# nju-websoft/OpenEA

Hardware: AMD Instinct MI355X
Metric: training triples/sec (k=10 truncated negatives + limited loss + Adagrad) (higher is better)
Workload: dtype f32; 1 GPU; BootEA/AlignE translational step, EN-FR-100K-V1 shape (synthetic), dim=100, GLOBAL batch=20000 positives (weak scaling: 20000 per GPU x 1 GPU), k=10, truncated eps=0.98; the same workload at every N (; global_batch=20000, entities=200000, parallelism=single

## Files before the change

include/openea_hip.h:

```cpp
#ifndef OPENEA_HIP_H
#define OPENEA_HIP_H

#include <stddef.h>
#include <stdint.h>

#ifdef __cplusplus
extern "C" {
#endif

#define OEA_OK 0
#define OEA_EINVAL (-1)
#define OEA_EHIP (-2)
#define OEA_ENOMEM (-3)
#define OEA_EUNSUPPORTED (-4)

int oea_version(void);
const char *oea_last_error(void);
int oea_device_count(void);

int oea_profile_begin(int32_t stride);
int oea_profile_end(int32_t group, double *out_ms_host, int32_t *n_calls_host);

typedef struct oea_store *oea_store_t;
int oea_store_create(int64_t rows, int32_t dim, oea_store_t *out);
// ... 298 lines not shown
    double *loss_accum;
} oea_epoch;
int oea_triple_epoch_range(const oea_epoch *e, int32_t step_begin, int32_t step_end, int32_t rank, int32_t world, void *plan,
                           size_t plan_bytes, int32_t plan_built, void *stream);

size_t oea_epoch_layout_bytes(int64_t n);
int oea_epoch_layout(const int32_t *triples, int64_t n1, int64_t n2, const int64_t *slot, int64_t n_slots, uint64_t seed, uint32_t epoch,
                     int32_t *dall, void *workspace, size_t ws_bytes, void *stream);

int32_t oea_step_plan_supported(const oea_step_cfg *cfg, int64_t n_ent, int64_t n_rel, int32_t ld, int32_t k);
size_t oea_step_plan_bytes(int64_t n_total, int32_t steps, int64_t max_batch, int64_t n_ent, int32_t ld);
int oea_step_plan_build(const int32_t *pos_all, const int32_t *neg_all, int32_t k, const int64_t *offsets_dev, int64_t n_total,
                        int32_t steps, int64_t max_batch, int64_t n_ent, int32_t ld, void *plan, size_t plan_bytes, void *stream);
int oea_step_plan_offsets(int64_t n_total, int32_t steps, int64_t max_batch, int64_t n_ent, int32_t ld, int64_t *out);
int oea_step_plan_rel_order_offset(int64_t n_total, int32_t steps, int64_t max_batch, int64_t n_ent, int32_t ld, int64_t *out);

struct oea_comm;
int oea_triple_epoch_range_comm(struct oea_comm *comm, const oea_epoch *e, int32_t step_begin, int32_t step_end, void *send, void *own,
                                void *rel_x, float *upd, float *all, void *stream);


uint32_t oea_perm_index(uint32_t i, uint32_t n, uint32_t key);
int oea_sample_link_negatives(const int32_t *pos_links, int64_t n_pos, int32_t k, const int32_t *ents1, int32_t n1,
                              const int32_t *ents2, int32_t n2, const int32_t *nbr1, const int32_t *row1,
                              const int32_t *nbr2, const int32_t *row2, int32_t nbr_k, const uint64_t *exclude,
                              uint64_t exclude_cap, uint64_t seed, uint32_t step, int32_t *out_pairs, float *out_valid,
                              uint64_t *scratch_keys, int32_t *scratch_vals, uint64_t scratch_cap, void *stream);

int oea_greedy_matching(const int32_t *left, const int32_t *right, const float *weight, int64_t n_edges,
                        uint8_t *selected);
// ... 243 lines not shown
```

openea_amd/_lib.py:

```python
import ctypes as C
import os

_HERE = os.path.dirname(os.path.abspath(__file__))
DETERMINISTIC = os.environ.get("OEA_STEP_DETERMINISTIC", "0")[:1] == "1"
LIB_PATH = os.environ.get("OPENEA_HIP_LIB") or os.path.join(_HERE, "csrc",
                                                            "libopenea_hip_det.so" if DETERMINISTIC else "libopenea_hip.so")


class OpenEAHipError(RuntimeError):
    pass


class StepCfg(C.Structure):
    _fields_ = [("loss_kind", C.c_int32), ("l1", C.c_int32), ("margin", C.c_float),
                ("pos_margin", C.c_float), ("neg_margin", C.c_float), ("balance", C.c_float),
                ("ent_l2_norm", C.c_int32), ("rel_l2_norm", C.c_int32), ("opt_kind", C.c_int32),
                ("lr", C.c_float), ("neg_group_k", C.c_int32), ("score_kind", C.c_int32),
                ("normal", C.c_void_p), ("normal_acc", C.c_void_p),
                ("ent_transfer_base", C.c_int32), ("rel_transfer_base", C.c_int32),
                ("beta1", C.c_float), ("beta2", C.c_float), ("eps", C.c_float), ("opt_t", C.c_int32)]


class SamplerSide(C.Structure):
    _fields_ = [("table", C.c_void_p), ("capacity", C.c_uint64), ("entity_list", C.c_void_p),
# ... 117 lines not shown
                                       _u32, _u32, _i32, _vp, _vp, _vp]),
    "oea_sample_negatives_replay": (C.c_int, [_vp, _i64, _i32, _vp, _u64, _vp, _i32, _vp, _vp, _i32, _i32, _vp, _vp, _vp, _vp]),
    "oea_tripleset_filter_bits": (C.c_uint64, [_u64]),
    "oea_tripleset_filter_build": (C.c_int, [_vp, _i64, _vp, _u64, _vp]),
    "oea_sample_negatives_pair": (C.c_int, [_vp, _i64, _i64, _i32, C.POINTER(SamplerSide), C.POINTER(SamplerSide),
                                            _u64, _u32, _u32, _i32, _vp, _vp, _vp]),
    "oea_sample_negatives_epoch": (C.c_int, [_vp, _i64, _vp, _vp, _i32, _i32, C.POINTER(SamplerSide),
                                             C.POINTER(SamplerSide), _u64, _u32, _i32, _vp, _vp, _vp]),
    "oea_triple_epoch_range": (C.c_int, [C.POINTER(Epoch), _i32, _i32, _i32, _i32, _vp, _sz, _i32, _vp]),
    "oea_epoch_layout_bytes": (_sz, [_i64]),
    "oea_epoch_layout": (C.c_int, [_vp, _i64, _i64, _vp, _i64, _u64, _u32, _vp, _vp, _sz, _vp]),
    "oea_step_plan_supported": (_i32, [C.POINTER(StepCfg), _i64, _i64, _i32, _i32]),
    "oea_step_plan_bytes": (_sz, [_i64, _i32, _i64, _i64, _i32]),
    "oea_step_plan_offsets": (C.c_int, [_i64, _i32, _i64, _i64, _i32, _vp]),
    "oea_step_plan_rel_order_offset": (C.c_int, [_i64, _i32, _i64, _i64, _i32, _vp]),
    "oea_step_plan_build": (C.c_int, [_vp, _vp, _i32, _vp, _i64, _i32, _i64, _i64, _i32, _vp, _sz, _vp]),
    "oea_triple_epoch_range_comm": (C.c_int, [_vp, C.POINTER(Epoch), _i32, _i32, _vp, _vp, _vp, _vp, _vp, _vp]),
    "oea_rotate_workspace_bytes": (_sz, [_i64, _i64, _i32]),
    "oea_rotate_exchange_doubles": (_sz, [_i64, _i64, _i32]),
    "oea_rotate_step": (C.c_int, [_vp, _vp, _i64, _vp, _vp, _i64, _i32, _i32, _vp, _i64, _vp, _i64, _i32,
                                  C.POINTER(RotateCfg), _vp, _vp, _i32, _vp]),
    "oea_rotate_lookup": (C.c_int, [_vp, _i64, _i32, _i32, _vp, _i64, _i32, _i32, _vp, _i32, _vp]),
    "oea_mapping_workspace_floats": (_sz, [_i64, _i32, _i32]),
    "oea_mapping_step": (C.c_int, [_vp, _i32, _i32, _i32, _vp, _vp, _i64, _vp, _vp, C.c_float, C.c_float, _i32, _vp, _vp,
                                   _vp, _vp, _vp]),
    "oea_mapping_epoch": (C.c_int, [_vp, _vp, _i64, _vp, _vp, _i64, _i32, _i32, _i32, _vp, _i32, _i64, _vp, _vp, _f32, _f32, _i32,
                                    C.POINTER(StepCfg), _vp, _vp, _vp, _vp, _vp]),
    "oea_sea_mapping_workspace_floats": (_sz, [_i64, _i64, _i32, _i32]),
    "oea_sea_mapping_step": (C.c_int, [_vp, _i32, _i32, _vp, _vp, _i64, _vp, _vp, _i64, _vp, _vp, _vp, _f32, _f32, C.POINTER(StepCfg),
                                       _vp, _vp, _vp, _vp, _vp]),
# ... 187 lines not shown
```

openea_amd/csrc/step_plan.h:

```cpp
#pragma once
#include <hip/hip_runtime.h>
#include <stddef.h>
#include <stdint.h>

namespace oea {

struct StepPlanView {
    uint64_t *keys_a, *keys_b;
    uint32_t *vals_a, *vals_b;
    uint64_t *ukeys;
    uint32_t *ucount;
    uint32_t *uoff;
    int32_t *n_unique;
    int32_t *step_first;
    uint32_t *pflags;
    uint4 *recs;
    uint8_t *inplan;
    float *contrib;
    void *temp;
    size_t temp_bytes;
    uint32_t *rel_order;
    int row_bits;
};

constexpr uint32_t kPlanHubEntries = 8;

size_t step_plan_layout(int64_t n_total, int32_t steps, int64_t max_batch, int64_t n_ent, int32_t ld, void *base, StepPlanView *v);

}
```

openea_amd/csrc/step_plan.hip:

```cpp
#include <string.h>

#include <rocprim/rocprim.hpp>

#include <algorithm>

#include "common.h"
#include "step_plan.h"

namespace oea {

static size_t al256(size_t x) { return (x + 255) / 256 * 256; }
static int bits_for(uint64_t max_value) { int b = 1; while (b < 64 && (max_value >> b) != 0) ++b; return b; }

size_t step_plan_layout(int64_t n_total, int32_t steps, int64_t max_batch, int64_t n_ent, int32_t ld, void *base, StepPlanView *v) {
    const size_t m = (size_t)std::max<int64_t>(2 * n_total, 1);
    size_t off = 0;
    char *b = static_cast<char *>(base);
    auto take = [&](size_t bytes) { size_t o = off; off += al256(bytes); return b ? b + o : nullptr; };
    StepPlanView w{};
    w.keys_a = (uint64_t *)take(8 * m);
    w.keys_b = (uint64_t *)take(8 * m);
    w.vals_a = (uint32_t *)take(4 * m);
    w.vals_b = (uint32_t *)take(4 * m);
    w.ukeys = (uint64_t *)take(8 * m);
// ... 4 lines not shown
    w.pflags = (uint32_t *)take(4 * (size_t)std::max<int64_t>(n_total, 1));
    w.recs = (uint4 *)take(16 * m);
    w.inplan = (uint8_t *)take((size_t)std::max<int32_t>(steps, 1) * (size_t)n_ent);
    w.contrib = (float *)take(sizeof(float) * 2 * (size_t)std::max<int64_t>(max_batch, 1) * (size_t)ld);
    size_t t1 = 0, t2 = 0, t3 = 0;
    (void)rocprim::radix_sort_pairs(nullptr, t1, (const uint64_t *)nullptr, (uint64_t *)nullptr, (const uint32_t *)nullptr,
                                    (uint32_t *)nullptr, m, 0, 64, (hipStream_t)0);
    (void)rocprim::run_length_encode(nullptr, t2, (const uint64_t *)nullptr, m, (uint64_t *)nullptr, (uint32_t *)nullptr,
                                     (int32_t *)nullptr, (hipStream_t)0);
    (void)rocprim::exclusive_scan(nullptr, t3, (const uint32_t *)nullptr, (uint32_t *)nullptr, 0u, m + 1, rocprim::plus<uint32_t>(),
                                  (hipStream_t)0);
    const size_t n1 = (size_t)std::max<int64_t>(n_total, 1);
    w.temp_bytes = std::max(std::max(t1, std::max(t2, t3)), al256(4 * n1)) + 256;
    w.temp = take(w.temp_bytes);
    w.rel_order = (uint32_t *)take(4 * n1);
    w.row_bits = bits_for((uint64_t)std::max<int64_t>(n_ent - 1, 1));
    if (v) *v = w;
    return off;
}

namespace {

__global__ void plan_emit_kernel(const int32_t *__restrict__ pos_all, const int32_t *__restrict__ neg_all, int k,
                                 const int64_t *__restrict__ offsets, int steps, int64_t n_total, int row_bits,
                                 uint64_t *__restrict__ keys, uint32_t *__restrict__ vals) {
    const int64_t p = (int64_t)blockIdx.x * blockDim.x + threadIdx.x;
    if (p >= n_total) return;
    int lo = 0, hi = steps;
    while (hi - lo > 1) {
        const int mid = (lo + hi) >> 1;
        if (offsets[mid] <= p) lo = mid; else hi = mid;
    }
    const uint32_t pl = (uint32_t)(p - offsets[lo]);
    const int h = pos_all[3 * p], r = pos_all[3 * p + 1], t = pos_all[3 * p + 2];
    unsigned bad = 0, xh = 0, xt = 0;
    const int32_t *ng = neg_all + p * k * 3;
    for (int j = 0; j < k; ++j) {
        const unsigned a = (unsigned)(ng[3 * j] ^ h), b = (unsigned)(ng[3 * j + 2] ^ t), c = (unsigned)(ng[3 * j + 1] ^ r);
        bad |= c | min(a, b);
        xh |= a;
        xt |= b;
    }
    if (bad | min(xh, xt)) {
        keys[2 * p] = keys[2 * p + 1] = (uint64_t)steps << row_bits;
        vals[2 * p] = vals[2 * p + 1] = 0u;
        return;
    }
    const bool tails = xh == 0;
    const uint64_t sk = (uint64_t)lo << row_bits;
    keys[2 * p] = sk | (uint64_t)(uint32_t)h;
    vals[2 * p] = 2u * pl + (tails ? 0u : 1u);
    keys[2 * p + 1] = sk | (uint64_t)(uint32_t)t;
    vals[2 * p + 1] = 0x80000000u | (2u * pl + (tails ? 1u : 0u));
}

constexpr int kRelSortWaves = 8, kRelDigitBits = 10, kRelBins = 1 << kRelDigitBits, kRelAhead = 8;
__global__ __launch_bounds__(kRelSortWaves * 64) void plan_rel_order_kernel(const int32_t *__restrict__ pos_all, const int64_t *__restrict__ offsets,
                                                                            uint32_t *__restrict__ tmp, uint32_t *__restrict__ rel_order) {
    __shared__ uint32_t hist[kRelSortWaves][kRelBins];
    __shared__ uint32_t dbase[kRelBins];
    __shared__ uint32_t wsum[kRelSortWaves];
    __shared__ uint32_t rmax;
    const int64_t first = offsets[blockIdx.x];
// ... 116 lines not shown
__global__ void plan_hub_kernel(const uint64_t *__restrict__ keys, const uint32_t *__restrict__ vals, int64_t m,
                                const int64_t *__restrict__ offsets, int steps, int row_bits, uint32_t *__restrict__ pflags) {
    const int64_t e = (int64_t)blockIdx.x * blockDim.x + threadIdx.x;
    if (e >= m) return;
    const uint64_t key = keys[e];
    const int64_t step = (int64_t)(key >> row_bits);
    if (step >= steps) return;
    int left = 0, right = 0;
    while (left < (int)kPlanHubEntries && e - left - 1 >= 0 && keys[e - left - 1] == key) ++left;
    while (left + right < (int)kPlanHubEntries && e + right + 1 < m && keys[e + right + 1] == key) ++right;
    if (left + right < (int)kPlanHubEntries) return;
    const uint32_t v = vals[e];
    atomicOr(&pflags[offsets[step] + ((v & 0x7fffffffu) >> 1)], (v >> 31) ? 2u : 1u);
}

__device__ __forceinline__ uint32_t mix32(uint32_t x) {
    x ^= x >> 16; x *= 0x7feb352du; x ^= x >> 15; x *= 0x846ca68bu; x ^= x >> 16;
    return x;
}
__device__ __forceinline__ uint32_t feistel_perm(uint32_t i, uint32_t n, int lbits, int rbits, const uint32_t (&key)[6]) {
    const uint32_t lmask = (1u << lbits) - 1u, rmask = (1u << rbits) - 1u;
    uint32_t x = i;
    do {
        uint32_t l = x >> rbits, r = x & rmask;
#pragma unroll
        for (int q = 0; q < 6; q += 2) {
            l = (l ^ mix32(r ^ key[q])) & lmask;
            r = (r ^ mix32(l ^ key[q + 1])) & rmask;
        }
        x = (l << rbits) | r;
// ... 32 lines not shown
    oea::StepPlanView v;
    char *base = reinterpret_cast<char *>(4096);
    const size_t total = oea::step_plan_layout(n_total, steps, max_batch, n_ent, ld, base, &v);
    out[0] = (char *)v.vals_b - base; out[1] = (char *)v.ukeys - base; out[2] = (char *)v.uoff - base;
    out[3] = (char *)v.n_unique - base; out[4] = (char *)v.step_first - base; out[5] = (char *)v.contrib - base;
    out[6] = v.row_bits; out[7] = (int64_t)total; out[8] = (char *)v.pflags - base;
    return OEA_OK;
}

int oea_step_plan_rel_order_offset(int64_t n_total, int32_t steps, int64_t max_batch, int64_t n_ent, int32_t ld, int64_t *out) {
    OEA_REQUIRE(out && n_total >= 0 && steps >= 0 && n_ent > 0 && ld > 0, "arguments");
    oea::StepPlanView v;
    char *base = reinterpret_cast<char *>(4096);
    (void)oea::step_plan_layout(n_total, steps, max_batch, n_ent, ld, base, &v);
    *out = (char *)v.rel_order - base;
    return OEA_OK;
}

size_t oea_epoch_layout_bytes(int64_t n) {
    return n < 0 ? 0 : 256;
}

int oea_epoch_layout(const int32_t *triples, int64_t n1, int64_t n2, const int64_t *slot, int64_t n_slots, uint64_t seed, uint32_t epoch,
                     int32_t *dall, void *workspace, size_t ws_bytes, void *stream) {
    OEA_REQUIRE(triples && (slot || n_slots == 0) && (dall || n_slots == 0), "null pointer");
    OEA_REQUIRE(n1 >= 0 && n2 >= 0 && n_slots >= 0 && n1 < ((int64_t)1 << 32) && n2 < ((int64_t)1 << 32), "sizes");
    (void)workspace; (void)ws_bytes;
    if (n1 + n2 == 0 || n_slots == 0) return OEA_OK;
    hipStream_t st = oea::as_stream(stream);
    oea::layout_perm_kernel<<<(unsigned)oea::ceil_div(n_slots, 256), 256, 0, st>>>(triples, n1, n2, slot, n_slots, (uint32_t)seed,
// ... 24 lines not shown
    size_t tb = v.temp_bytes;
    OEA_CHECK_HIP(rocprim::radix_sort_pairs(v.temp, tb, (const uint64_t *)v.keys_a, v.keys_b, (const uint32_t *)v.vals_a, v.vals_b, m, 0,
                                            (unsigned)end_bit, st));
    OEA_CHECK_HIP(hipMemsetAsync(v.ucount, 0, sizeof(uint32_t) * (m + 1), st));
    tb = v.temp_bytes;
    OEA_CHECK_HIP(rocprim::run_length_encode(v.temp, tb, (const uint64_t *)v.keys_b, m, v.ukeys, v.ucount, v.n_unique, st));
    tb = v.temp_bytes;
    OEA_CHECK_HIP(rocprim::exclusive_scan(v.temp, tb, (const uint32_t *)v.ucount, v.uoff, 0u, m + 1, rocprim::plus<uint32_t>(), st));
    oea::plan_step_first_kernel<<<(unsigned)oea::ceil_div(steps + 1, 256), 256, 0, st>>>(v.ukeys, v.n_unique, steps, v.row_bits, v.step_first);
    OEA_CHECK_HIP(hipMemsetAsync(v.pflags, 0, sizeof(uint32_t) * (size_t)n_total, st));
    OEA_CHECK_HIP(hipMemsetAsync(v.inplan, 0, (size_t)steps * (size_t)n_ent, st));
    oea::plan_records_kernel<<<(unsigned)std::min<int64_t>(oea::ceil_div((int64_t)m, 256), 4096), 256, 0, st>>>(
        v.ukeys, v.uoff, v.vals_b, v.n_unique, steps, v.row_bits, n_ent, v.recs, v.inplan);
    oea::plan_hub_kernel<<<(unsigned)oea::ceil_div((int64_t)m, 256), 256, 0, st>>>(v.keys_b, v.vals_b, (int64_t)m, offsets_dev, steps, v.row_bits,
                                                                                   v.pflags);
    OEA_CHECK_HIP(hipGetLastError());
    return OEA_OK;
}

}
```

openea_amd/csrc/triple_step.hip:

```cpp
#include <stdlib.h>

#include <algorithm>
#include <type_traits>
#include <vector>

#include "common.h"
#include "step_plan.h"

namespace {

using oea::align256;
using oea::group_sum;

using oea::flag_t;
using oea::grad_t;

struct StepWs {
    grad_t *ent_grad, *rel_grad;
    grad_t *rel_extra;
    int64_t rel_copy_stride;
    flag_t *ent_touched, *rel_touched;
    grad_t *nrm_grad, *nrm_extra;
    flag_t *nrm_touched;
    double *partials;
// ... 429 lines not shown

template <int IT>
__device__ __forceinline__ void wave_normalize(Row<64, IT> &r) {
    float s = 0.f;
#pragma unroll
    for (int it = 0; it < IT; ++it) s += r.v[it] * r.v[it];
    const float inv = rsqrtf(fmaxf(oea::wave_sum_uniform(s), 1e-12f));
#pragma unroll
    for (int it = 0; it < IT; ++it) r.v[it] *= inv;
}

template <int IT, int L1, int KT, bool PLAN>
__global__ __launch_bounds__(512, (IT <= 2 ? (KT == 10 ? 8 : 7) : 4)) void triple_wave(
    const float *__restrict__ ent, const float *__restrict__ rel, int ld, const int32_t *__restrict__ pos,
    int64_t n_pos, const int32_t *__restrict__ neg, int k, oea_step_cfg cfg, StepWs ws, int dbg, float *__restrict__ contrib,
    const uint32_t *__restrict__ pflags, const uint32_t *__restrict__ order) {
    constexpr int G = 64, KC = 10;
    if (KT > 0) k = KT;
    const int lane = threadIdx.x & 63;
    const int wv = __builtin_amdgcn_readfirstlane((int)(threadIdx.x >> 6));
    const int wpb = blockDim.x >> 6;
    const int64_t nw = (int64_t)gridDim.x * wpb;
    const int row_b = ld * 4, row_g = ld << kGradShift;
    const __amdgpu_buffer_rsrc_t rs_ent = __builtin_amdgcn_make_buffer_rsrc(const_cast<float *>(ent), 0, (dbg & 2) ? 0 : kBufRecords, kBufFlags);
    const __amdgpu_buffer_rsrc_t rs_rel = __builtin_amdgcn_make_buffer_rsrc(const_cast<float *>(rel), 0, (dbg & 2) ? 0 : kBufRecords, kBufFlags);
    const __amdgpu_buffer_rsrc_t rs_eg = __builtin_amdgcn_make_buffer_rsrc(ws.ent_grad, 0, (dbg & 1) ? 0 : kBufRecords, kBufFlags);
    const __amdgpu_buffer_rsrc_t rs_et = __builtin_amdgcn_make_buffer_rsrc(ws.ent_touched, 0, (dbg & 4) ? 0 : kBufRecords, kBufFlags);
    const int v4 = lane * 4, vg = lane << kGradShift;
    const int c_last = (IT - 1) * 64 + lane;
    const int vt = c_last < ld ? c_last * 4 : kBufOob, vgt = c_last < ld ? c_last << kGradShift : kBufOob;
    const float c_neg = L1 ? -cfg.balance : -2.f * cfg.balance;
    double loss_local = 0.0;
    auto score_positive = [&](int64_t p, Row<G, IT> &gacc) -> int {
        const int32_t *pp = pos + 3 * p;
        const int32_t *ng = neg + p * k * 3;
        const int h = pp[0], r = pp[1], t = pp[2];
        Row<G, IT> yh, yr, yt;
        wave_load_row<IT>(rs_ent, h * row_b, v4, vt, yh);
        wave_load_row<IT>(rs_rel, r * row_b, v4, vt, yr);
        wave_load_row<IT>(rs_ent, t * row_b, v4, vt, yt);
        int ids[3 * KC];
        if (KT == KC || k == KC) {
#pragma unroll
            for (int q = 0; q < 3 * KC; ++q) ids[q] = ng[q];
        } else {
#pragma unroll
            for (int q = 0; q < 3 * KC; ++q) ids[q] = q < 3 * k ? ng[q] : 0;
        }
        unsigned bad = 0, xh = 0, xt = 0;
#pragma unroll
        for (int j = 0; j < KC; ++j)
            if (KT == KC || j < k) {
                const unsigned a = (unsigned)(ids[3 * j] ^ h), b = (unsigned)(ids[3 * j + 2] ^ t), c = (unsigned)(ids[3 * j + 1] ^ r);
                bad |= c | min(a, b);
                xh |= a;
                xt |= b;
            }
        if (bad) {
            double ls = score_independent<G, IT>(ent, rel, ld, lane, p, h, r, t, true, cfg, ws, OEA_LOSS_LIMITED, L1);
#pragma unroll 1
            for (int j = 0; j < k; ++j)
                ls += score_independent<G, IT>(ent, rel, ld, lane, p, ng[3 * j], ng[3 * j + 1], ng[3 * j + 2], false, cfg, ws, OEA_LOSS_LIMITED, L1);
            loss_local = uniform_d(loss_local + ls);
            return -1;
        }
        if (min(xh, xt)) {
            unsigned tmask = 0;
            int ce[KC];
            Row<G, IT> yc[KC];
#pragma unroll
            for (int j = 0; j < KC; ++j)
                if (KT == KC || j < k) {
                    const int nh = ids[3 * j], nt = ids[3 * j + 2];
                    const bool tl = nh == h;
                    tmask |= tl ? 1u << j : 0u;
                    ce[j] = tl ? nt : nh;
                    wave_load_row<IT>(rs_ent, ce[j] * row_b, v4, vt, yc[j]);
                }
            asm volatile("" : "+s"(tmask));
#pragma unroll
            for (int it = 0; it < IT; ++it)
                asm volatile("" : "+v"(yh.v[it]), "+v"(yr.v[it]), "+v"(yt.v[it]));
            wave_normalize<IT>(yh);
            wave_normalize<IT>(yr);
            wave_normalize<IT>(yt);
            Row<G, IT> u, gpos;
            float sp = 0.f;
#pragma unroll
            for (int it = 0; it < IT; ++it) {
                u.v[it] = yh.v[it] + yr.v[it];
                const float d = u.v[it] - yt.v[it];
                gpos.v[it] = d;
                sp += L1 ? fabsf(d) : d * d;
// ... 45 lines not shown
                        wave_atomic_row<IT>(rs_eg, pe * row_g, vg, vgt, g, -sign_c);
                        buf_flag_set(rs_et, pe);
                    }
                }
            if (cpos) {
                wave_atomic_row<IT>(rs_eg, h * row_g, vg, vgt, gpos, 1.f);
                buf_flag_set(rs_et, h);
                wave_atomic_row<IT>(rs_eg, t * row_g, vg, vgt, gpos, -1.f);
                buf_flag_set(rs_et, t);
            }
            loss_local = uniform_d(loss_local + (double)lsum);
            if (!(cpos | anyneg)) return -1;
            if (PLAN && order) return r;
            wave_rel_row<IT>(ws, dbg, p, r, row_g, vg, vgt, gacc);
            return -1;
        }
        auto one_sided = [&](auto side) -> int {
            constexpr bool tails = decltype(side)::value;
            int ce[KC];
            Row<G, IT> yc[KC];
#pragma unroll
            for (int j = 0; j < KC; ++j)
                if (KT == KC || j < k) {
                    ce[j] = tails ? ids[3 * j + 2] : ids[3 * j];
                    wave_load_row<IT>(rs_ent, ce[j] * row_b, v4, vt, yc[j]);
                }
            wave_normalize<IT>(yh);
            wave_normalize<IT>(yr);
            wave_normalize<IT>(yt);
            Row<G, IT> u, gpos;
            int r_sum = -1;
            float sp = 0.f;
#pragma unroll
            for (int it = 0; it < IT; ++it) {
                u.v[it] = yh.v[it] + yr.v[it];
                const float d = u.v[it] - yt.v[it];
                gpos.v[it] = d;
                sp += L1 ? fabsf(d) : d * d;
            }
            const float xp = oea::wave_sum_uniform(sp) - cfg.pos_margin;
            const bool cpos = xp > 0.f;
// ... 53 lines not shown
                    }
                }
            if (PLAN) {
                const __amdgpu_buffer_rsrc_t rs_cb = __builtin_amdgcn_make_buffer_rsrc(contrib, 0, kBufRecords, kBufFlags);
                const int so = (int)p * 2 * row_b;
#pragma unroll
                for (int it = 0; it < IT; ++it) {
                    const int vo = it < IT - 1 ? v4 + it * 256 : vt;
                    __builtin_amdgcn_raw_buffer_store_b32(__builtin_bit_cast(unsigned, gacc.v[it]), rs_cb, vo, so, 0);
                    __builtin_amdgcn_raw_buffer_store_b32(__builtin_bit_cast(unsigned, gpos.v[it]), rs_cb, vo, so + row_b, 0);
                }
            }
            if (cpos | anyneg) {
                if (PLAN && order) r_sum = r;
                else wave_rel_row<IT>(ws, dbg, p, r, row_g, vg, vgt, gacc);
                const unsigned via_atomics = PLAN ? pflags[p] : 3u;
                const bool h_full = tails, t_full = !tails;
                if ((via_atomics & 1u) && (h_full || cpos)) {
                    wave_atomic_row<IT>(rs_eg, h * row_g, vg, vgt, h_full ? gacc : gpos, 1.f);
                    buf_flag_set(rs_et, h);
                }
                if ((via_atomics & 2u) && (t_full || cpos)) {
                    wave_atomic_row<IT>(rs_eg, t * row_g, vg, vgt, t_full ? gacc : gpos, -1.f);
                    buf_flag_set(rs_et, t);
                }
            }
            loss_local = uniform_d(loss_local + (double)lsum);
            return r_sum;
        };
        return xh == 0 ? one_sided(std::true_type{}) : one_sided(std::false_type{});
    };
    if constexpr (!PLAN) {
        for (int64_t p = (int64_t)blockIdx.x * wpb + wv; p < n_pos; p += nw) {
            Row<G, IT> gacc;
            (void)score_positive(p, gacc);
        }
    } else {
        for (int64_t q0 = (int64_t)blockIdx.x * wpb; q0 < n_pos; q0 += nw) {
            const int64_t q = q0 + wv;
            Row<G, IT> gacc;
            const int r_sum = q < n_pos ? score_positive(order ? (int64_t)order[q] : q, gacc) : -1;
            if (!order) continue;
            __shared__ float s_row[8][IT][64];
            __shared__ int s_rel[8];
            int lb = v4;
            asm volatile("" : "+v"(lb));
            const auto at = [lb](auto *base) { return (decltype(base))((char *)base + lb); };
            if (lb == 0) s_rel[wv] = r_sum;
            if (r_sum >= 0) {
#pragma unroll
                for (int it = 0; it < IT; ++it) *at(&s_row[wv][it][0]) = gacc.v[it];
            }
            __syncthreads();
            if (r_sum >= 0) {
                const int held = lb < wpb * 4 ? *at(&s_rel[0]) : -1;
                bool first = true;
#pragma unroll
                for (int w = 0; w < 8; ++w) first = first && !(w < wv && __builtin_amdgcn_readlane(held, w) == r_sum);
                if (first) {
#pragma unroll
                    for (int w = 1; w < 8; ++w)
                        if (w > wv && __builtin_amdgcn_readlane(held, w) == r_sum) {
#pragma unroll
                            for (int it = 0; it < IT; ++it) gacc.v[it] += *at(&s_row[w][it][0]);
                        }
                    wave_rel_row<IT>(ws, dbg, order[q], r_sum, row_g, vg, vgt, gacc);
                }
            }
            if (q0 + nw < n_pos) __syncthreads();
        }
    }
    __shared__ double sred[8];
    int lz = v4;
    if constexpr (PLAN) asm volatile("" : "+v"(lz));
    if (lz == 0) sred[wv] = loss_local;
    __syncthreads();
    if (wv == 0 && lz == 0) {
        double s = 0.0;
        for (int w = 0; w < wpb; ++w) s += sred[w];
        ws.partials[blockIdx.x] = s;
    }
// ... 1044 lines not shown
    for (int64_t i = (int64_t)blockIdx.x * blockDim.x + threadIdx.x; i < total; i += (int64_t)gridDim.x * blockDim.x) {
        const int64_t j = i / cpr, id = j * world + rank;
        const int c = (int)(i - j * cpr);
        oea::st4(upd + j * ld + 4 * c, id < n_ent ? oea::ld4(ent + id * ld + 4 * c) : make_float4(0.f, 0.f, 0.f, 0.f));
    }
}

static bool step_wave_enabled() {
    static const int env = [] { const char *e = getenv("OEA_STEP_WAVE"); return e ? atoi(e) : 1; }();
    return env != 0;
}

template <int IT64>
void launch_wave(int nb, int block, hipStream_t st, const float *ent, const float *rel, int ld, const int32_t *pos,
                 int64_t n_pos, const int32_t *neg, const oea_step_cfg &cfg, const StepWs &ws, float *contrib = nullptr,
                 const uint32_t *pflags = nullptr, const uint32_t *order = nullptr) {
    const int k = cfg.neg_group_k;
    static const int dbg = [] { const char *e = getenv("OEA_STEP_WAVE_DBG"); return e ? atoi(e) : 0; }();
#define OEA_WAVE(L1, KT)                                                                                                               \
    do {                                                                                                                               \
        if constexpr (!oea::kDetScratch) {                                    \
            if (contrib) {                                                                                                             \
                oea::launch_timed(triple_wave<IT64, L1, KT, true>, nb, block, st, ent, rel, ld, pos, n_pos, neg, k, cfg, ws, dbg, contrib, pflags, order);   \
                break;                                                                                                                 \
            }                                                                                                                          \
        }                                                                                                                              \
        oea::launch_timed(triple_wave<IT64, L1, KT, false>, nb, block, st, ent, rel, ld, pos, n_pos, neg, k, cfg, ws, dbg, contrib, pflags, nullptr);   \
    } while (0)
    if (k == 10) { if (cfg.l1) OEA_WAVE(1, 10); else OEA_WAVE(0, 10); }
    else { if (cfg.l1) OEA_WAVE(1, 0); else OEA_WAVE(0, 0); }
#undef OEA_WAVE
}

static bool step_runtime_kind() {
    static const int env = [] { const char *e = getenv("OEA_STEP_RUNTIME_KIND"); return e ? atoi(e) : 0; }();
    return env != 0;
}

static bool wave_rule(const oea_step_cfg &cfg, int64_t n_ent, int64_t n_rel, int32_t ld) {
    return cfg.score_kind == OEA_SCORE_TRANSE && cfg.loss_kind == OEA_LOSS_LIMITED && cfg.ent_l2_norm && cfg.rel_l2_norm &&
           cfg.neg_group_k >= 1 && cfg.neg_group_k <= 10 && ld <= 256 &&
           std::max(n_ent, n_rel) * (int64_t)ld * (int64_t)sizeof(grad_t) < ((int64_t)1 << 30) && step_wave_enabled() &&
           !step_runtime_kind();
}

template <int G, int IT>
constexpr bool kWaveInstance = (G == 32 && IT <= 4) || (G == 64 && IT == 4);
template <int G, int IT>
constexpr bool kPlanInstance = kWaveInstance<G, IT> && !oea::kDetScratch;

template <int G, int IT>
void launch_grouped(int nb, int block, hipStream_t st, const float *ent, const float *rel, int ld, const int32_t *pos,
                    int64_t n_pos, const int32_t *neg, const oea_step_cfg &cfg, const StepWs &ws, bool wave, float *contrib = nullptr,
                    const uint32_t *pflags = nullptr, const uint32_t *order = nullptr) {
    const bool runtime_kind = step_runtime_kind();
    const int k = cfg.neg_group_k;
    if constexpr (kWaveInstance<G, IT>) {
        if (wave) {
            constexpr int IT64 = G == 32 ? (IT + 1) / 2 : 4;
            static const int blk_env = [] { const char *e = getenv("OEA_STEP_WAVE_BLOCK"); return e ? atoi(e) : 0; }();
            const int wblock = G == 32 ? (blk_env == 256 || blk_env == 512 ? blk_env : 512) : (block / G) * 64;
            launch_wave<IT64>(nb, wblock, st, ent, rel, ld, pos, n_pos, neg, cfg, ws, contrib, pflags, order);
            return;
        }
    }
#define OEA_GROUPED(LOSS, L1) oea::launch_timed(triple_grouped<G, IT, LOSS, L1>, nb, block, st, ent, rel, ld, pos, n_pos, neg, k, cfg, ws)
    if (runtime_kind) OEA_GROUPED(-1, -1);
    else if (cfg.loss_kind == OEA_LOSS_LIMITED) { if (cfg.l1) OEA_GROUPED(OEA_LOSS_LIMITED, 1); else OEA_GROUPED(OEA_LOSS_LIMITED, 0); }
    else if (cfg.loss_kind == OEA_LOSS_LOGISTIC) { if (cfg.l1) OEA_GROUPED(OEA_LOSS_LOGISTIC, 1); else OEA_GROUPED(OEA_LOSS_LOGISTIC, 0); }
    else if (cfg.loss_kind == OEA_LOSS_POSITIVE) { if (cfg.l1) OEA_GROUPED(OEA_LOSS_POSITIVE, 1); else OEA_GROUPED(OEA_LOSS_POSITIVE, 0); }
    else OEA_GROUPED(-1, -1);
#undef OEA_GROUPED
}

static bool apply_g16(int64_t n_ent, int64_t n_rel, int32_t ld) {
    static const int env_g16 = [] { const char *e = getenv("OEA_APPLY_G16"); return e ? atoi(e) : -1; }();
    return env_g16 >= 0 ? env_g16 != 0 : (n_ent + n_rel) * (int64_t)ld * 12 > (int64_t)128 << 20;
// ... 51 lines not shown
    const bool projected = transd || (transh && !transh_grouped);
    const bool grouped = transh_grouped || (!projected && cfg.neg_group_k > 0 && cfg.loss_kind != OEA_LOSS_MARGIN);
    const int64_t items = step_items(cfg, n_pos, n_neg);
    const int n_part = loss_partials(ld, items);
    const int nb1 = std::max(n_part, 1);
    if (phase != OEA_PHASE_APPLY) {
        oea::prof_call();
        if (transd)
            oea::launch_timed(triple_projected<G, IT, OEA_SCORE_TRANSD>, nb1, block, st, ent, rel, ld, pos, n_pos, neg, n_neg, cfg, ws);
        else if (projected)
            oea::launch_timed(triple_projected<G, IT, OEA_SCORE_TRANSH>, nb1, block, st, ent, rel, ld, pos, n_pos, neg, n_neg, cfg, ws);
        else if (transh)
            oea::launch_timed(triple_transh_grouped<G, IT>, nb1, block, st, ent, rel, ld, pos, n_pos, neg, n_neg ? cfg.neg_group_k : 0, cfg, ws);
        else if (grouped) {
            static const bool rel_order_on = [] { const char *e = getenv("OEA_STEP_REL_ORDER"); return !(e && e[0] == '0'); }();
            launch_grouped<G, IT>(nb1, block, st, ent, rel, ld, pos, n_pos, neg, cfg, ws, wave_rule(cfg, n_ent, n_rel, ld),
                                  plan ? plan->contrib : nullptr, plan ? plan->pflags + plan_first_pos : nullptr,
                                  plan && rel_order_on ? plan->rel_order + plan_first_pos : nullptr);
        }
        else
            oea::launch_timed(triple_generic<G, IT>, nb1, block, st, ent, rel, ld, pos, n_pos, neg, n_neg, cfg, ws);
        if (phase == OEA_PHASE_GRAD || dense_opt)
            fold_rel_copies_kernel<<<(unsigned)std::min<int64_t>(oea::ceil_div(n_rel * (int64_t)ld, 256), 1024), 256, 0, st>>>(
                ws, n_rel * (int64_t)ld, transh ? 1 : 0);
    }
    const int nb2 = (int)std::min<int64_t>(std::max<int64_t>(oea::ceil_div(n_ent + n_rel, gpb), 1), 16384);
    if (phase != OEA_PHASE_GRAD) {
        hipEvent_t ev0 = nullptr, ev1 = nullptr;
        (void)oea::prof_pair(&ev0, &ev1);
        if (dense_opt) {
            const double t = (double)cfg.opt_t;
            const float lr_t = cfg.opt_kind == OEA_OPT_ADAM
                                   ? (float)((double)cfg.lr * std::sqrt(1.0 - std::pow((double)cfg.beta2, t)) / (1.0 - std::pow((double)cfg.beta1, t)))
// ... 613 lines not shown
```

openea_amd/ops.py:

```python
import ctypes as C
import math
import os

import numpy as np
import torch

from . import _lib
from ._lib import LOSS_KIND, METRIC, OPT_KIND, OpenEAHipError, RotateCfg, StepCfg, check


def lib():
    return _lib.load(require_device=True)


def _p(t):
    if t is None:
        return None
    assert t.is_cuda and t.is_contiguous(), "device-resident contiguous tensor required"
    return C.c_void_p(t.data_ptr())


def _stream():
    return C.c_void_p(torch.cuda.current_stream().cuda_stream)

# ... 940 lines not shown
    check(lib().oea_step_plan_offsets(int(n_total), int(steps), int(max_batch), int(n_ent), int(ld), C.cast(off, C.c_void_p)))
    raw = plan.cpu().numpy()
    m = 2 * int(n_total)
    nu = int(raw[off[3]: off[3] + 4].view(np.int32)[0])
    return dict(vals=raw[off[0]: off[0] + 4 * m].view(np.uint32).copy(), ukeys=raw[off[1]: off[1] + 8 * nu].view(np.uint64).copy(),
                uoff=raw[off[2]: off[2] + 4 * (nu + 1)].view(np.uint32).copy(),
                step_first=raw[off[4]: off[4] + 4 * (steps + 1)].view(np.int32).copy(), row_bits=int(off[6]), n_unique=nu,
                pflags=raw[off[8]: off[8] + 4 * int(n_total)].view(np.uint32).copy())


def step_plan_rel_order(plan, n_total, steps, max_batch, n_ent, ld):
    off = C.c_int64(0)
    check(lib().oea_step_plan_rel_order_offset(int(n_total), int(steps), int(max_batch), int(n_ent), int(ld), C.cast(C.byref(off), C.c_void_p)))
    n = int(n_total)
    return plan[off.value: off.value + 4 * n].cpu().numpy().view(np.uint32).copy()


def step_plan_stats(plan, n_total, steps, max_batch, n_ent, ld):
    a = step_plan_arrays(plan, n_total, steps, max_batch, n_ent, ld)
    last = int(a["step_first"][steps])
    cnt = np.diff(a["uoff"].astype(np.int64))[:last]
    listed = int(a["uoff"][last])
    hub = cnt > 8
    return dict(positives=int(n_total), outside_rule=int(n_total - listed // 2), rows_per_step=float(last) / max(steps, 1),
                refs_per_row_mean=float(cnt.mean()) if last else 0.0, refs_per_row_max=int(cnt.max()) if last else 0,
                hub_rows_per_step=float(hub.sum()) / max(steps, 1), refs_to_hub_rows=int(cnt[hub].sum()),
                refs_listed=listed)


def comm_single_or_none():
# ... 782 lines not shown
```

Measured before the change: 293.5 million triples/s.

## Precompute per-slot 64-byte records in step plan for wave kernel

Adds a plan-build kernel that packs, for each slot in relation order, the positive id, hub flags, rule kind, tail mask, h/r/t and the ten corrupted entity ids into a 16-word record. The wave scoring kernel then reads one aligned 64-byte vector per slot instead of an order indirection, a scattered positive triple load, 30 negative ids and a pflags lookup, and it no longer recomputes the rule classification. The cost is extra plan memory and build time, plus a kernel refactor into foreign/mixed/one_sided lambdas, which may change register pressure.

```diff
diff --git a/include/openea_hip.h b/include/openea_hip.h
--- a/include/openea_hip.h
+++ b/include/openea_hip.h
@@ -336,6 +336,7 @@
                         int32_t steps, int64_t max_batch, int64_t n_ent, int32_t ld, void *plan, size_t plan_bytes, void *stream);
 int oea_step_plan_offsets(int64_t n_total, int32_t steps, int64_t max_batch, int64_t n_ent, int32_t ld, int64_t *out);
 int oea_step_plan_rel_order_offset(int64_t n_total, int32_t steps, int64_t max_batch, int64_t n_ent, int32_t ld, int64_t *out);
+int oea_step_plan_slot_rec_offset(int64_t n_total, int32_t steps, int64_t max_batch, int64_t n_ent, int32_t ld, int64_t *out);
 
 struct oea_comm;
 int oea_triple_epoch_range_comm(struct oea_comm *comm, const oea_epoch *e, int32_t step_begin, int32_t step_end, void *send, void *own,
diff --git a/openea_amd/_lib.py b/openea_amd/_lib.py
--- a/openea_amd/_lib.py
+++ b/openea_amd/_lib.py
@@ -155,6 +155,7 @@
     "oea_step_plan_bytes": (_sz, [_i64, _i32, _i64, _i64, _i32]),
     "oea_step_plan_offsets": (C.c_int, [_i64, _i32, _i64, _i64, _i32, _vp]),
     "oea_step_plan_rel_order_offset": (C.c_int, [_i64, _i32, _i64, _i64, _i32, _vp]),
+    "oea_step_plan_slot_rec_offset": (C.c_int, [_i64, _i32, _i64, _i64, _i32, _vp]),
     "oea_step_plan_build": (C.c_int, [_vp, _vp, _i32, _vp, _i64, _i32, _i64, _i64, _i32, _vp, _sz, _vp]),
     "oea_triple_epoch_range_comm": (C.c_int, [_vp, C.POINTER(Epoch), _i32, _i32, _vp, _vp, _vp, _vp, _vp, _vp]),
     "oea_rotate_workspace_bytes": (_sz, [_i64, _i64, _i32]),
diff --git a/openea_amd/csrc/step_plan.h b/openea_amd/csrc/step_plan.h
--- a/openea_amd/csrc/step_plan.h
+++ b/openea_amd/csrc/step_plan.h
@@ -20,8 +20,31 @@
     void *temp;
     size_t temp_bytes;
     uint32_t *rel_order;
+    uint32_t *slot_rec;
     int row_bits;
 };
+
+struct PlanRule {
+    unsigned bad = 0, xh = 0, xt = 0;
+};
+__host__ __device__ __forceinline__ void plan_rule_add(PlanRule &u, int h, int r, int t, int nh, int nr, int nt) {
+    const unsigned a = (unsigned)(nh ^ h), b = (unsigned)(nt ^ t), c = (unsigned)(nr ^ r);
+    u.bad |= c | (a < b ? a : b);
+    u.xh |= a;
+    u.xt |= b;
+}
+enum : unsigned {
+    kPlanTails = 0,
+    kPlanHeads = 1,
+    kPlanMixed = 2,
+    kPlanForeign = 3
+};
+__host__ __device__ __forceinline__ unsigned plan_rule_kind(const PlanRule &u) {
+    return u.bad ? kPlanForeign : (u.xh < u.xt ? u.xh : u.xt) ? kPlanMixed : u.xh ? kPlanHeads : kPlanTails;
+}
+
+constexpr int kSlotRecWords = 16, kSlotRecNegs = 10;
+constexpr int kSlotRecIds = 2, kSlotRecCe = 5, kSlotRecKindShift = 2, kSlotRecMaskShift = 4;
 
 constexpr uint32_t kPlanHubEntries = 8;
 
diff --git a/openea_amd/csrc/step_plan.hip b/openea_amd/csrc/step_plan.hip
--- a/openea_amd/csrc/step_plan.hip
+++ b/openea_amd/csrc/step_plan.hip
@@ -42,6 +42,7 @@
     w.temp_bytes = std::max(std::max(t1, std::max(t2, t3)), al256(4 * n1)) + 256;
     w.temp = take(w.temp_bytes);
     w.rel_order = (uint32_t *)take(4 * n1);
+    w.slot_rec = (uint32_t *)take(4 * (size_t)kSlotRecWords * n1);
     w.row_bits = bits_for((uint64_t)std::max<int64_t>(n_ent - 1, 1));
     if (v) *v = w;
     return off;
@@ -61,20 +62,16 @@
     }
     const uint32_t pl = (uint32_t)(p - offsets[lo]);
     const int h = pos_all[3 * p], r = pos_all[3 * p + 1], t = pos_all[3 * p + 2];
-    unsigned bad = 0, xh = 0, xt = 0;
+    PlanRule rule;
     const int32_t *ng = neg_all + p * k * 3;
-    for (int j = 0; j < k; ++j) {
-        const unsigned a = (unsigned)(ng[3 * j] ^ h), b = (unsigned)(ng[3 * j + 2] ^ t), c = (unsigned)(ng[3 * j + 1] ^ r);
-        bad |= c | min(a, b);
-        xh |= a;
-        xt |= b;
-    }
-    if (bad | min(xh, xt)) {
+    for (int j = 0; j < k; ++j) plan_rule_add(rule, h, r, t, ng[3 * j], ng[3 * j + 1], ng[3 * j + 2]);
+    const unsigned kind = plan_rule_kind(rule);
+    if (kind >= kPlanMixed) {
         keys[2 * p] = keys[2 * p + 1] = (uint64_t)steps << row_bits;
         vals[2 * p] = vals[2 * p + 1] = 0u;
         return;
     }
-    const bool tails = xh == 0;
+    const bool tails = kind == kPlanTails;
     const uint64_t sk = (uint64_t)lo << row_bits;
     keys[2 * p] = sk | (uint64_t)(uint32_t)h;
     vals[2 * p] = 2u * pl + (tails ? 0u : 1u);
@@ -221,6 +218,48 @@
     atomicOr(&pflags[offsets[step] + ((v & 0x7fffffffu) >> 1)], (v >> 31) ? 2u : 1u);
 }
 
+constexpr int kSlotRecLanes = 16, kSlotRecBlock = 256;
+static_assert(kSlotRecLanes == kSlotRecWords && kSlotRecNegs <= kSlotRecLanes, "one lane per word, and a lane for every negative");
+__global__ __launch_bounds__(kSlotRecBlock) void plan_slot_rec_kernel(const int32_t *__restrict__ pos_all, const int32_t *__restrict__ neg_all, int k,
+                                                                      const int64_t *__restrict__ offsets, uint32_t bps,
+                                                                      const uint32_t *__restrict__ rel_order, const uint32_t *__restrict__ pflags,
+                                                                      uint32_t *__restrict__ slot_rec) {
+    const uint32_t s = blockIdx.x / bps;
+    const int64_t first = offsets[s], n = offsets[s + 1] - first;
+    const int64_t q = (int64_t)(blockIdx.x - s * bps) * (kSlotRecBlock / kSlotRecLanes) + (threadIdx.x / kSlotRecLanes);
+    if (q >= n) return;
+    const int l = (int)(threadIdx.x % kSlotRecLanes);
+    const uint32_t p = rel_order[first + q];
+    const int64_t gp = first + p;
+    const int h = pos_all[3 * gp], r = pos_all[3 * gp + 1], t = pos_all[3 * gp + 2];
+    const bool on = l < k;
+    int nh = h, nr = r, nt = t;
+    if (on) {
+        const int32_t *ng = neg_all + (gp * k + l) * 3;
+        nh = ng[0]; nr = ng[1]; nt = ng[2];
+    }
+    PlanRule u;
+    plan_rule_add(u, h, r, t, nh, nr, nt);
+    unsigned keeps = on && nh == h ? 1u << l : 0u;
+    for (int o = kSlotRecLanes / 2; o > 0; o >>= 1) {
+        u.bad |= (unsigned)__shfl_xor((int)u.bad, o, kSlotRecLanes);
+        u.xh |= (unsigned)__shfl_xor((int)u.xh, o, kSlotRecLanes);
+        u.xt |= (unsigned)__shfl_xor((int)u.xt, o, kSlotRecLanes);
+        keeps |= (unsigned)__shfl_xor((int)keeps, o, kSlotRecLanes);
+    }
+    const unsigned kind = plan_rule_kind(u);
+    const int ce = !on ? 0 : kind == kPlanTails ? nt : kind == kPlanHeads ? nh : (nh == h ? nt : nh);
+    const int ce_l = __shfl(ce, (l + kSlotRecLanes - kSlotRecCe) % kSlotRecLanes, kSlotRecLanes);
+    uint32_t w = 0u;
+    if (l == 0) w = p;
+    else if (l == 1) w = pflags[gp] | kind << kSlotRecKindShift | (kind == kPlanMixed ? keeps << kSlotRecMaskShift : 0u);
+    else if (l == kSlotRecIds) w = (uint32_t)h;
+    else if (l == kSlotRecIds + 1) w = (uint32_t)r;
+    else if (l == kSlotRecIds + 2) w = (uint32_t)t;
+    else if (l < kSlotRecCe + kSlotRecNegs) w = (uint32_t)ce_l;
+    slot_rec[(first + q) * kSlotRecWords + l] = w;
+}
+
 __device__ __forceinline__ uint32_t mix32(uint32_t x) {
     x ^= x >> 16; x *= 0x7feb352du; x ^= x >> 15; x *= 0x846ca68bu; x ^= x >> 16;
     return x;
@@ -283,6 +322,29 @@
     char *base = reinterpret_cast<char *>(4096);
     (void)oea::step_plan_layout(n_total, steps, max_batch, n_ent, ld, base, &v);
     *out = (char *)v.rel_order - base;
+    return OEA_OK;
+}
+
+int oea_step_plan_slot_rec_offset(int64_t n_total, int32_t steps, int64_t max_batch, int64_t n_ent, int32_t ld, int64_t *out) {
+    OEA_REQUIRE(out && n_total >= 0 && steps >= 0 && n_ent > 0 && ld > 0, "arguments");
+    oea::StepPlanView v;
+    char *base = reinterpret_cast<char *>(4096);
+    (void)oea::step_plan_layout(n_total, steps, max_batch, n_ent, ld, base, &v);
+    *out = (char *)v.slot_rec - base;
+    return OEA_OK;
+}
+
+int oea_step_plan_rule_kinds(const int32_t *pos, const int32_t *neg, int32_t k, int64_t n, uint32_t *kinds) {
+    OEA_REQUIRE((pos && kinds) || n == 0, "null pointer");
+    OEA_REQUIRE(n >= 0 && k >= 0 && (neg || k == 0 || n == 0), "sizes");
+    for (int64_t i = 0; i < n; ++i) {
+        oea::PlanRule u;
+        for (int j = 0; j < k; ++j) {
+            const int32_t *g = neg + (i * k + j) * 3;
+            oea::plan_rule_add(u, pos[3 * i], pos[3 * i + 1], pos[3 * i + 2], g[0], g[1], g[2]);
+        }
+        kinds[i] = oea::plan_rule_kind(u);
+    }
     return OEA_OK;
 }
 
@@ -337,6 +399,12 @@
         v.ukeys, v.uoff, v.vals_b, v.n_unique, steps, v.row_bits, n_ent, v.recs, v.inplan);
     oea::plan_hub_kernel<<<(unsigned)oea::ceil_div((int64_t)m, 256), 256, 0, st>>>(v.keys_b, v.vals_b, (int64_t)m, offsets_dev, steps, v.row_bits,
                                                                                    v.pflags);
+    if (k <= oea::kSlotRecNegs && max_batch > 0) {
+        const int64_t bps = oea::ceil_div(max_batch, (int64_t)(oea::kSlotRecBlock / oea::kSlotRecLanes));
+        OEA_REQUIRE(bps * steps < ((int64_t)1 << 31), "slot record grid");
+        oea::plan_slot_rec_kernel<<<(unsigned)(bps * steps), oea::kSlotRecBlock, 0, st>>>(pos_all, neg_all, k, offsets_dev, (uint32_t)bps,
+                                                                                        v.rel_order, v.pflags, v.slot_rec);
+    }
     OEA_CHECK_HIP(hipGetLastError());
     return OEA_OK;
 }
diff --git a/openea_amd/csrc/triple_step.hip b/openea_amd/csrc/triple_step.hip
--- a/openea_amd/csrc/triple_step.hip
+++ b/openea_amd/csrc/triple_step.hip
@@ -467,8 +467,10 @@
 __global__ __launch_bounds__(512, (IT <= 2 ? (KT == 10 ? 8 : 7) : 4)) void triple_wave(
     const float *__restrict__ ent, const float *__restrict__ rel, int ld, const int32_t *__restrict__ pos,
     int64_t n_pos, const int32_t *__restrict__ neg, int k, oea_step_cfg cfg, StepWs ws, int dbg, float *__restrict__ contrib,
-    const uint32_t *__restrict__ pflags, const uint32_t *__restrict__ order) {
+    const uint32_t *__restrict__ pflags, const uint32_t *__restrict__ order, const uint32_t *__restrict__ srec) {
     constexpr int G = 64, KC = 10;
+    static_assert(KC == oea::kSlotRecNegs, "a slot record holds KC corrupted entities");
+    if constexpr (!(PLAN && IT <= 2)) srec = nullptr;
     if (KT > 0) k = KT;
     const int lane = threadIdx.x & 63;
     const int wv = __builtin_amdgcn_readfirstlane((int)(threadIdx.x >> 6));
@@ -484,52 +486,22 @@
     const int vt = c_last < ld ? c_last * 4 : kBufOob, vgt = c_last < ld ? c_last << kGradShift : kBufOob;
     const float c_neg = L1 ? -cfg.balance : -2.f * cfg.balance;
     double loss_local = 0.0;
-    auto score_positive = [&](int64_t p, Row<G, IT> &gacc) -> int {
-        const int32_t *pp = pos + 3 * p;
+    auto foreign = [&](int64_t p, int h, int r, int t) __attribute__((always_inline)) -> int {
         const int32_t *ng = neg + p * k * 3;
-        const int h = pp[0], r = pp[1], t = pp[2];
-        Row<G, IT> yh, yr, yt;
-        wave_load_row<IT>(rs_ent, h * row_b, v4, vt, yh);
-        wave_load_row<IT>(rs_rel, r * row_b, v4, vt, yr);
-        wave_load_row<IT>(rs_ent, t * row_b, v4, vt, yt);
-        int ids[3 * KC];
-        if (KT == KC || k == KC) {
-#pragma unroll
-            for (int q = 0; q < 3 * KC; ++q) ids[q] = ng[q];
-        } else {
-#pragma unroll
-            for (int q = 0; q < 3 * KC; ++q) ids[q] = q < 3 * k ? ng[q] : 0;
-        }
-        unsigned bad = 0, xh = 0, xt = 0;
-#pragma unroll
-        for (int j = 0; j < KC; ++j)
-            if (KT == KC || j < k) {
-                const unsigned a = (unsigned)(ids[3 * j] ^ h), b = (unsigned)(ids[3 * j + 2] ^ t), c = (unsigned)(ids[3 * j + 1] ^ r);
-                bad |= c | min(a, b);
-                xh |= a;
-                xt |= b;
-            }
-        if (bad) {
-            double ls = score_independent<G, IT>(ent, rel, ld, lane, p, h, r, t, true, cfg, ws, OEA_LOSS_LIMITED, L1);
+        double ls = score_independent<G, IT>(ent, rel, ld, lane, p, h, r, t, true, cfg, ws, OEA_LOSS_LIMITED, L1);
 #pragma unroll 1
-            for (int j = 0; j < k; ++j)
-                ls += score_independent<G, IT>(ent, rel, ld, lane, p, ng[3 * j], ng[3 * j + 1], ng[3 * j + 2], false, cfg, ws, OEA_LOSS_LIMITED, L1);
-            loss_local = uniform_d(loss_local + ls);
-            return -1;
-        }
-        if (min(xh, xt)) {
-            unsigned tmask = 0;
-            int ce[KC];
+        for (int j = 0; j < k; ++j)
+            ls += score_independent<G, IT>(ent, rel, ld, lane, p, ng[3 * j], ng[3 * j + 1], ng[3 * j + 2], false, cfg, ws, OEA_LOSS_LIMITED, L1);
+        loss_local = uniform_d(loss_local + ls);
+        return -1;
+    };
+    auto mixed = [&](int64_t p, int h, int r, int t, unsigned tmask, const int (&ce)[KC], Row<G, IT> &yh, Row<G, IT> &yr, Row<G, IT> &yt,
+                     Row<G, IT> &gacc) __attribute__((always_inline)) -> int {
             Row<G, IT> yc[KC];
 #pragma unroll
             for (int j = 0; j < KC; ++j)
-                if (KT == KC || j < k) {
-                    const int nh = ids[3 * j], nt = ids[3 * j + 2];
-                    const bool tl = nh == h;
-                    tmask |= tl ? 1u << j : 0u;
-                    ce[j] = tl ? nt : nh;
-                    wave_load_row<IT>(rs_ent, ce[j] * row_b, v4, vt, yc[j]);
-                }
+                if (KT == KC || j < k) wave_load_row<IT>(rs_ent, ce[j] * row_b, v4, vt, yc[j]);
+            if constexpr (KT == 0) tmask = (unsigned)__builtin_amdgcn_readfirstlane((int)tmask);
             asm volatile("" : "+s"(tmask));
 #pragma unroll
             for (int it = 0; it < IT; ++it)
@@ -605,17 +577,14 @@
             if (PLAN && order) return r;
             wave_rel_row<IT>(ws, dbg, p, r, row_g, vg, vgt, gacc);
             return -1;
-        }
-        auto one_sided = [&](auto side) -> int {
+    };
+    auto one_sided = [&](auto side, int64_t p, int h, int r, int t, const int (&ce)[KC], auto hub, Row<G, IT> &yh, Row<G, IT> &yr,
+                         Row<G, IT> &yt, Row<G, IT> &gacc) __attribute__((always_inline)) -> int {
             constexpr bool tails = decltype(side)::value;
-            int ce[KC];
             Row<G, IT> yc[KC];
 #pragma unroll
             for (int j = 0; j < KC; ++j)
-                if (KT == KC || j < k) {
-                    ce[j] = tails ? ids[3 * j + 2] : ids[3 * j];
-                    wave_load_row<IT>(rs_ent, ce[j] * row_b, v4, vt, yc[j]);
-                }
+                if (KT == KC || j < k) wave_load_row<IT>(rs_ent, ce[j] * row_b, v4, vt, yc[j]);
             wave_normalize<IT>(yh);
             wave_normalize<IT>(yr);
             wave_normalize<IT>(yt);
@@ -699,7 +668,7 @@
             if (cpos | anyneg) {
                 if (PLAN && order) r_sum = r;
                 else wave_rel_row<IT>(ws, dbg, p, r, row_g, vg, vgt, gacc);
-                const unsigned via_atomics = PLAN ? pflags[p] : 3u;
+                const unsigned via_atomics = PLAN ? hub() : 3u;
                 const bool h_full = tails, t_full = !tails;
                 if ((via_atomics & 1u) && (h_full || cpos)) {
                     wave_atomic_row<IT>(rs_eg, h * row_g, vg, vgt, h_full ? gacc : gpos, 1.f);
@@ -712,10 +681,74 @@
             }
             loss_local = uniform_d(loss_local + (double)lsum);
             return r_sum;
-        };
-        return xh == 0 ? one_sided(std::true_type{}) : one_sided(std::false_type{});
+    };
+    auto score_positive = [&](int64_t p, Row<G, IT> &gacc) -> int {
+        const int32_t *pp = pos + 3 * p;
+        const int32_t *ng = neg + p * k * 3;
+        const int h = pp[0], r = pp[1], t = pp[2];
+        Row<G, IT> yh, yr, yt;
+        wave_load_row<IT>(rs_ent, h * row_b, v4, vt, yh);
+        wave_load_row<IT>(rs_rel, r * row_b, v4, vt, yr);
+        wave_load_row<IT>(rs_ent, t * row_b, v4, vt, yt);
+        int ids[3 * KC];
+        if (KT == KC || k == KC) {
+#pragma unroll
+            for (int q = 0; q < 3 * KC; ++q) ids[q] = ng[q];
+        } else {
+#pragma unroll
+            for (int q = 0; q < 3 * KC; ++q) ids[q] = q < 3 * k ? ng[q] : 0;
+        }
+        oea::PlanRule rule;
+#pragma unroll
+        for (int j = 0; j < KC; ++j)
+            if (KT == KC || j < k) oea::plan_rule_add(rule, h, r, t, ids[3 * j], ids[3 * j + 1], ids[3 * j + 2]);
+        const unsigned kind = oea::plan_rule_kind(rule);
+        if (kind == oea::kPlanForeign) return foreign(p, h, r, t);
+        int ce[KC];
+        if (kind == oea::kPlanMixed) {
+            unsigned tmask = 0;
+#pragma unroll
+            for (int j = 0; j < KC; ++j)
+                if (KT == KC || j < k) {
+                    const int nh = ids[3 * j], nt = ids[3 * j + 2];
+                    const bool tl = nh == h;
+                    tmask |= tl ? 1u << j : 0u;
+                    ce[j] = tl ? nt : nh;
+                }
+            return mixed(p, h, r, t, tmask, ce, yh, yr, yt, gacc);
+        }
+        const auto hub = [&]() -> unsigned { return pflags[p]; };
+        if (kind == oea::kPlanTails) {
+#pragma unroll
+            for (int j = 0; j < KC; ++j) ce[j] = ids[3 * j + 2];
+            return one_sided(std::true_type{}, p, h, r, t, ce, hub, yh, yr, yt, gacc);
+        }
+#pragma unroll
+        for (int j = 0; j < KC; ++j) ce[j] = ids[3 * j];
+        return one_sided(std::false_type{}, p, h, r, t, ce, hub, yh, yr, yt, gacc);
+    };
+    auto score_slot = [&](const uint32_t *__restrict__ rec, Row<G, IT> &gacc) -> int {
+        typedef uint32_t rec_t __attribute__((ext_vector_type(oea::kSlotRecWords)));
+        const rec_t w = *reinterpret_cast<const rec_t *>(rec);
+        const int64_t p = (int64_t)w[0];
+        const unsigned flags = w[1], kind = (flags >> oea::kSlotRecKindShift) & 3u;
+        const int h = (int)w[oea::kSlotRecIds], r = (int)w[oea::kSlotRecIds + 1], t = (int)w[oea::kSlotRecIds + 2];
+        if (kind == oea::kPlanForeign) return foreign(p, h, r, t);
+        Row<G, IT> yh, yr, yt;
+        wave_load_row<IT>(rs_ent, h * row_b, v4, vt, yh);
+        wave_load_row<IT>(rs_rel, r * row_b, v4, vt, yr);
+        wave_load_row<IT>(rs_ent, t * row_b, v4, vt, yt);
+        int ce[KC];
+#pragma unroll
+        for (int j = 0; j < KC; ++j) ce[j] = (int)w[oea::kSlotRecCe + j];
+        if (kind == oea::kPlanMixed)
+            return mixed(p, h, r, t, (flags >> oea::kSlotRecMaskShift) & ((1u << KC) - 1u), ce, yh, yr, yt, gacc);
+        const auto hub = [&]() -> unsigned { return flags & 3u; };
+        if (kind == oea::kPlanTails) return one_sided(std::true_type{}, p, h, r, t, ce, hub, yh, yr, yt, gacc);
+        return one_sided(std::false_type{}, p, h, r, t, ce, hub, yh, yr, yt, gacc);
     };
     if constexpr (!PLAN) {
+        (void)score_slot;
         for (int64_t p = (int64_t)blockIdx.x * wpb + wv; p < n_pos; p += nw) {
             Row<G, IT> gacc;
             (void)score_positive(p, gacc);
@@ -724,7 +757,9 @@
         for (int64_t q0 = (int64_t)blockIdx.x * wpb; q0 < n_pos; q0 += nw) {
             const int64_t q = q0 + wv;
             Row<G, IT> gacc;
-            const int r_sum = q < n_pos ? score_positive(order ? (int64_t)order[q] : q, gacc) : -1;
+            const int r_sum = q >= n_pos ? -1
+                              : srec     ? score_slot((const uint32_t *)__builtin_assume_aligned(srec + q * oea::kSlotRecWords, 64), gacc)
+                                         : score_positive(order ? (int64_t)order[q] : q, gacc);
             if (!order) continue;
             __shared__ float s_row[8][IT][64];
             __shared__ int s_rel[8];
@@ -749,7 +784,7 @@
 #pragma unroll
                             for (int it = 0; it < IT; ++it) gacc.v[it] += *at(&s_row[w][it][0]);
                         }
-                    wave_rel_row<IT>(ws, dbg, order[q], r_sum, row_g, vg, vgt, gacc);
+                    wave_rel_row<IT>(ws, dbg, srec ? (int64_t)srec[q * oea::kSlotRecWords] : (int64_t)order[q], r_sum, row_g, vg, vgt, gacc);
                 }
             }
             if (q0 + nw < n_pos) __syncthreads();
@@ -1824,18 +1859,18 @@
 template <int IT64>
 void launch_wave(int nb, int block, hipStream_t st, const float *ent, const float *rel, int ld, const int32_t *pos,
                  int64_t n_pos, const int32_t *neg, const oea_step_cfg &cfg, const StepWs &ws, float *contrib = nullptr,
-                 const uint32_t *pflags = nullptr, const uint32_t *order = nullptr) {
+                 const uint32_t *pflags = nullptr, const uint32_t *order = nullptr, const uint32_t *srec = nullptr) {
     const int k = cfg.neg_group_k;
     static const int dbg = [] { const char *e = getenv("OEA_STEP_WAVE_DBG"); return e ? atoi(e) : 0; }();
 #define OEA_WAVE(L1, KT)                                                                                                               \
     do {                                                                                                                               \
         if constexpr (!oea::kDetScratch) {                                    \
             if (contrib) {                                                                                                             \
-                oea::launch_timed(triple_wave<IT64, L1, KT, true>, nb, block, st, ent, rel, ld, pos, n_pos, neg, k, cfg, ws, dbg, contrib, pflags, order);   \
+                oea::launch_timed(triple_wave<IT64, L1, KT, true>, nb, block, st, ent, rel, ld, pos, n_pos, neg, k, cfg, ws, dbg, contrib, pflags, order, srec);   \
                 break;                                                                                                                 \
             }                                                                                                                          \
         }                                                                                                                              \
-        oea::launch_timed(triple_wave<IT64, L1, KT, false>, nb, block, st, ent, rel, ld, pos, n_pos, neg, k, cfg, ws, dbg, contrib, pflags, nullptr);   \
+        oea::launch_timed(triple_wave<IT64, L1, KT, false>, nb, block, st, ent, rel, ld, pos, n_pos, neg, k, cfg, ws, dbg, contrib, pflags, nullptr, nullptr);   \
     } while (0)
     if (k == 10) { if (cfg.l1) OEA_WAVE(1, 10); else OEA_WAVE(0, 10); }
     else { if (cfg.l1) OEA_WAVE(1, 0); else OEA_WAVE(0, 0); }
@@ -1862,7 +1897,7 @@
 template <int G, int IT>
 void launch_grouped(int nb, int block, hipStream_t st, const float *ent, const float *rel, int ld, const int32_t *pos,
                     int64_t n_pos, const int32_t *neg, const oea_step_cfg &cfg, const StepWs &ws, bool wave, float *contrib = nullptr,
-                    const uint32_t *pflags = nullptr, const uint32_t *order = nullptr) {
+                    const uint32_t *pflags = nullptr, const uint32_t *order = nullptr, const uint32_t *srec = nullptr) {
     const bool runtime_kind = step_runtime_kind();
     const int k = cfg.neg_group_k;
     if constexpr (kWaveInstance<G, IT>) {
@@ -1870,7 +1905,7 @@
             constexpr int IT64 = G == 32 ? (IT + 1) / 2 : 4;
             static const int blk_env = [] { const char *e = getenv("OEA_STEP_WAVE_BLOCK"); return e ? atoi(e) : 0; }();
             const int wblock = G == 32 ? (blk_env == 256 || blk_env == 512 ? blk_env : 512) : (block / G) * 64;
-            launch_wave<IT64>(nb, wblock, st, ent, rel, ld, pos, n_pos, neg, cfg, ws, contrib, pflags, order);
+            launch_wave<IT64>(nb, wblock, st, ent, rel, ld, pos, n_pos, neg, cfg, ws, contrib, pflags, order, srec);
             return;
         }
     }
@@ -1952,9 +1987,12 @@
             oea::launch_timed(triple_transh_grouped<G, IT>, nb1, block, st, ent, rel, ld, pos, n_pos, neg, n_neg ? cfg.neg_group_k : 0, cfg, ws);
         else if (grouped) {
             static const bool rel_order_on = [] { const char *e = getenv("OEA_STEP_REL_ORDER"); return !(e && e[0] == '0'); }();
+            static const bool slot_rec_on = [] { const char *e = getenv("OEA_STEP_SLOT_REC"); return !(e && e[0] == '0'); }();
+            const bool recs = plan && rel_order_on && slot_rec_on && cfg.neg_group_k <= oea::kSlotRecNegs;
             launch_grouped<G, IT>(nb1, block, st, ent, rel, ld, pos, n_pos, neg, cfg, ws, wave_rule(cfg, n_ent, n_rel, ld),
                                   plan ? plan->contrib : nullptr, plan ? plan->pflags + plan_first_pos : nullptr,
-                                  plan && rel_order_on ? plan->rel_order + plan_first_pos : nullptr);
+                                  plan && rel_order_on ? plan->rel_order + plan_first_pos : nullptr,
+                                  recs ? plan->slot_rec + plan_first_pos * oea::kSlotRecWords : nullptr);
         }
         else
             oea::launch_timed(triple_generic<G, IT>, nb1, block, st, ent, rel, ld, pos, n_pos, neg, n_neg, cfg, ws);
diff --git a/openea_amd/ops.py b/openea_amd/ops.py
--- a/openea_amd/ops.py
+++ b/openea_amd/ops.py
@@ -978,6 +978,13 @@
     check(lib().oea_step_plan_rel_order_offset(int(n_total), int(steps), int(max_batch), int(n_ent), int(ld), C.cast(C.byref(off), C.c_void_p)))
     n = int(n_total)
     return plan[off.value: off.value + 4 * n].cpu().numpy().view(np.uint32).copy()
+
+
+def step_plan_slot_records(plan, n_total, steps, max_batch, n_ent, ld):
+    off = C.c_int64(0)
+    check(lib().oea_step_plan_slot_rec_offset(int(n_total), int(steps), int(max_batch), int(n_ent), int(ld), C.cast(C.byref(off), C.c_void_p)))
+    n = int(n_total)
+    return plan[off.value: off.value + 64 * n].cpu().numpy().view(np.uint32).reshape(n, 16).copy()
 
 
 def step_plan_stats(plan, n_total, steps, max_batch, n_ent, ld):
```

Measured after the change: 288.0 million triples/s. 0.981x the previous value.
